# SJTU-IPADS/wukong

Hardware: AMD Instinct MI355X
Metric: queries/sec, LUBM-2560 Q1-Q7 mix (OSDI16 plans) (higher is better)
Workload: dtype u32

## Files before the change

wukong_amd/csrc/gpu_engine.hip:

```cpp
#include "wk_store.h"
#include "../../include/wukong_abi.h"

#include <hip/hip_runtime.h>

#include <vector>
#include <algorithm>
#include <cstring>
#include <cstdio>
#include <cstdlib>
#include <chrono>
#include <type_traits>

static double now_us() {
    return std::chrono::duration<double, std::micro>(
               std::chrono::steady_clock::now().time_since_epoch()).count();
}
static int wk_verbose_lvl() {
    static int v = -1;
    if (v < 0) { const char *e = getenv("WK_VERBOSE"); v = e ? atoi(e) : 0; }
    return v;
}

using namespace wk;

// ... 138 lines not shown
    int nvars = 0;
    int step = 0;
    struct fconj { std::vector<wk_fnode_t> prog; int after; };
    std::vector<wk_fnode_t> filt;
    std::vector<fconj> conj;

    struct wk_graph {
        hipGraphExec_t exec = nullptr;
        std::vector<int32_t> v2c;
        int ncols = 0, cur = 0, nvars = 0;
        int64_t bound = 0;
        bool light = false;
        const sid_t *view = nullptr;
        bool fin = false;
        fin_sig_t fin_sig;
    };
    std::vector<wk_graph> graphs;
    int capturing = 0;
    std::vector<uint8_t> capture_hint;
    int capture_empty_after = -1;

    bool timing = false;
    std::vector<timed_launch> pending;
    double cat_usec[CAT_COUNT] = {0};
    double cat_bytes[CAT_COUNT] = {0};
    int64_t cat_n[CAT_COUNT] = {0};

    int var2col(ssid_t v) const { return v < 0 ? v2c[-(v + 1)] : -1; }
    int var_stat(ssid_t v) const { return v >= 0 ? 2 : (var2col(v) >= 0 ? 1 : 0); }
};

static const int BLOCK = 256;
static_assert(BLOCK == SCAN_T, "kernels declare __launch_bounds__(SCAN_T)");
static inline const sid_t *cur_table(wk_engine *e);
static int grid_for(int64_t work) {
    int64_t g = (work + BLOCK - 1) / BLOCK;
    return (int)(g < 1 ? 1 : (g > 2048 ? 2048 : g));
}
static inline const sid_t *cur_table(wk_engine *e) {
    return e->tbl_view ? e->tbl_view : (const sid_t *)e->tbl[e->cur].p;
}
static int32_t materialize_view(wk_engine *e) {
    if (!e->tbl_view) return WK_OK;
    size_t bytes = (size_t)std::max<int64_t>(e->nrows, 0) *
                   std::max(e->ncols, 1) * 4;
    if (bytes &&
        hipMemcpyAsync(e->tbl[e->cur].p, e->tbl_view, bytes,
                       hipMemcpyDeviceToDevice, e->stream) != hipSuccess)
        return WK_ERR_HIP;
    e->tbl_view = nullptr;
    return WK_OK;
}
static inline void fin_invalidate(wk_engine *e) {
    e->fin_count = -1;
    e->fin_table = false;
}
static int fin_grid(int64_t cap_rows) {
    int64_t g = (cap_rows + BLOCK - 1) / BLOCK;
    return (int)(g < 1 ? 1 : (g > FIN_MAXB ? FIN_MAXB : g));
}
static int scan_grid(int64_t bound) {
    int64_t g = (bound + SCAN_T) / SCAN_T + 1;
    return (int)(g < 1 ? 1 : (g > 2048 ? 2048 : g));
}

static hipEvent_t ev_get() { hipEvent_t e; (void)hipEventCreate(&e); return e; }

static bool wk_fn_dispatch() {
    const char *v = getenv("WK_FN_DISPATCH");
    return !(v && !atoi(v));
}

static bool wk_row_chain() {
    const char *v = getenv("WK_ROW_CHAIN");
    return !(v && v[0] == '0');
}
static bool wk_chain() {
    const char *v = getenv("WK_CHAIN");
    return !(v && !atoi(v));
}
static bool chain_narrow(int out_cols) {
    const char *v = getenv("WK_CHAIN_WIDTH");
    return out_cols <= ROW_NARROW && !(v && atoi(v) == ROW_MAX);
}
static bool wk_filter_batch() {
    const char *v = getenv("WK_FILTER_BATCH");
    return !(v && !atoi(v));
}
static bool wk_wave_scan() {
    const char *v = getenv("WK_SCAN");
    return !(v && !atoi(v));
}

static bool wk_filter_pushdown() {
    const char *v = getenv("WK_FILTER_PUSHDOWN");
    return !(v && !atoi(v));
}

static bool wk_spin_sync() {
    static int v = -1;
    if (v < 0) { const char *e = getenv("WK_SPIN_SYNC"); v = e ? atoi(e) : 0; }
    return v;
}
static hipError_t stream_sync(hipStream_t s) {
    if (!wk_spin_sync()) return hipStreamSynchronize(s);
    hipError_t rc;
    while ((rc = hipStreamQuery(s)) == hipErrorNotReady) {}
    return rc;
}

#define TIME_BEGIN(eng)                                                     \
    hipEvent_t t_s_ = nullptr, t_e_ = nullptr;                              \
    if ((eng)->timing && !(eng)->capturing) {                               \
        t_s_ = ev_get(); t_e_ = ev_get();                                   \
        (void)hipEventRecord(t_s_, (eng)->stream); }

#define TIME_END(eng, category)                                             \
    if ((eng)->timing && !(eng)->capturing) {                               \
        (void)hipEventRecord(t_e_, (eng)->stream);                          \
        (eng)->pending.push_back({t_s_, t_e_, (category)}); }

static const char *CAT_NAMES[CAT_COUNT] = {"probe", "scan", "expand", "filter",
                                           "copy", "split", "other"};

static void resolve_timing(wk_engine *e) {
    for (auto &t : e->pending) {
        float ms = 0;
        (void)hipEventElapsedTime(&ms, t.start, t.stop);
        if (wk_verbose_lvl() >= 3)
            fprintf(stderr, "[launch] %s %.0fus\n", CAT_NAMES[t.cat], ms * 1e3);
        e->cat_usec[t.cat] += ms * 1000.0;
        e->cat_n[t.cat]++;
        (void)hipEventDestroy(t.start);
        (void)hipEventDestroy(t.stop);
    }
    e->pending.clear();
}

static int64_t min_cap_rows() {
    const char *v = getenv("WK_MIN_CAP");
    return v ? atoll(v) : (1 << 20);
}

static int32_t grow_caps(wk_engine *e, int64_t rows, int cols) {
    rows = std::max<int64_t>(rows, min_cap_rows());
    cols = std::max(cols, std::max(e->cap_cols, 1));
    if (rows <= e->cap_rows && cols <= e->cap_cols) return WK_OK;
    if (e->capturing) return WK_ERR_STATE;
    rows = std::max(rows, e->cap_rows);
    HIP_CHECK(stream_sync(e->stream));
    fin_invalidate(e);
    size_t keep = (size_t)std::max<int64_t>(e->nrows, 0) * std::max(e->ncols, 0) * 4;
    keep = std::min(keep, e->tbl[e->cur].cap);
    void *saved = nullptr;
    if (keep) {
        if (hipMalloc(&saved, keep) != hipSuccess) return WK_ERR_HIP;
        HIP_CHECK(hipMemcpy(saved, e->tbl[e->cur].p, keep, hipMemcpyDeviceToDevice));
    }
    if (e->tbl[0].ensure((size_t)rows * cols * 4)) return WK_ERR_HIP;
    if (e->tbl[1].ensure((size_t)rows * cols * 4)) return WK_ERR_HIP;
    if (saved) {
        HIP_CHECK(hipMemcpy(e->tbl[e->cur].p, saved, keep, hipMemcpyDeviceToDevice));
        (void)hipFree(saved);
    }
    if (e->cnt.ensure((size_t)(rows + 1) * 4)) return WK_ERR_HIP;
    if (e->pmask.ensure((size_t)(rows + 1) * 4)) return WK_ERR_HIP;
// ... 519 lines not shown
    if (e->h_pin[S_ERR]) {
        e->h_pin[7] = 0;
        return WK_ERR_CAP;
    }
    return WK_OK;
}

static int32_t sync_state_grow(wk_engine *e) {
    int32_t rc = sync_state(e);
    if (rc != WK_ERR_CAP) return rc;
    int64_t need = (int64_t)e->h_pin[S_REQ];
    e->nrows = 0;
    int32_t rc2 = grow_caps(e, need + need / 4, e->cap_cols);
    if (rc2) return rc2;
    e->zero_pending = true;
    return WK_ERR_CAP;
}

template <class F>
static void with_ncols(int ncols, F &&f) {
    switch (ncols) {
    case 1: f(std::integral_constant<int, 1>{}); break;
    case 2: f(std::integral_constant<int, 2>{}); break;
    case 3: f(std::integral_constant<int, 3>{}); break;
    case 4: f(std::integral_constant<int, 4>{}); break;
    case 5: f(std::integral_constant<int, 5>{}); break;
    case 6: f(std::integral_constant<int, 6>{}); break;
    case 7: f(std::integral_constant<int, 7>{}); break;
    default: f(std::integral_constant<int, 8>{}); break;
    }
}


static bool hint_nodrop(const wk_engine *e, int step) {
    return e->capturing && step < (int)e->capture_hint.size() &&
           e->capture_hint[step];
}

static sid_t typeof_lookahead(const wk_engine *e, ssid_t o) {
    if (e->step + 1 >= (int)e->pats.size()) return 0;
    const wk_pattern_t &nx = e->pats[e->step + 1];
    if (nx.subject == o && nx.predicate == (ssid_t)TYPE_ID &&
        nx.direction == DIR_OUT && nx.object > 0)
        return (sid_t)nx.object;
    return 0;
}

static const uint64_t *type_bitmap(const wk_engine *e, sid_t type_id) {
    return (e->gs && (size_t)type_id < e->gs->d_tbm.size())
               ? e->gs->d_tbm[type_id]
               : nullptr;
}

static const fnpage_t *fn_map(const wk_engine *e, ssid_t p, int dir,
                              const sid_t **vals) {
    const size_t w = (size_t)p * 2 + dir;
    if (!e->gs || w >= e->gs->d_fn_pages.size() || !e->gs->d_fn_pages[w])
        return nullptr;
    *vals = e->gs->d_fn_vals[w];
    return e->gs->d_fn_pages[w];
}

struct chain_plan {
    chain_t C{};
    int npat = 0;
    int nfilter = 0;
    int out_cols = 0;
    int nnew = 0;
    ssid_t new_vars[CHAIN_MAX];
    bool lone_typeof(int col) const {
        return npat == 1 && C.op[0].kind == CH_TYPE && C.op[0].a == col;
    }
};

static bool chain_enabled(const wk_engine *e) {
    return e->whole_plan && !e->hinting && !e->opt_mode &&
           e->remote_step_idx < 0 && e->gs && wk_fn_dispatch() && wk_chain();
}

static void collect_chain(const wk_engine *e, int from,
                          std::vector<int32_t> v2c, int ncols,
                          chain_plan &cp) {
    const wk_store *st = e->st;
    cp.C.fn_base = st->fn_base;
    cp.C.fn_n = st->fn_n;
    cp.C.t_base = st->type_base;
    cp.C.t_n = st->type_n;
    int end = (int)e->pats.size();
    if (e->capturing && e->capture_empty_after >= 0)
        end = std::min(end, e->capture_empty_after + 1);
    auto col_of = [&](ssid_t v) {
        const int i = -(v + 1);
        return (v < 0 && i < (int)v2c.size()) ? v2c[i] : -1;
    };
    for (int i = from; i < end && cp.npat < CHAIN_MAX; i++) {
        const wk_pattern_t &pt = e->pats[i];
        const ssid_t p = pt.predicate;
        const int dir = pt.direction;
        const int a = col_of(pt.subject);
        if (a < 0 || p < 1) break;
        if ((sid_t)p == TYPE_ID && dir == DIR_IN) break;
        chain_op op{nullptr, nullptr, 0, a, 0, 0};
        const sid_t *vals = nullptr;
        if (pt.object >= 0) {
            if ((sid_t)p == TYPE_ID && dir == DIR_OUT) {
                const uint64_t *tbm = type_bitmap(e, (sid_t)pt.object);
                if (!tbm) break;
                op.kind = CH_TYPE;
                op.data = tbm;
            } else {
                if (fn_map(e, p, dir, &vals) || st->nsrv != 1 ||
                    !fn_map(e, p, dir ^ 1, &vals))
                    break;
                op.kind = CH_EQ;
                op.cval = st->fn_get((size_t)p * 2 + (dir ^ 1),
                                     (sid_t)pt.object);
            }
            cp.nfilter++;
        } else if (col_of(pt.object) >= 0) {
            op.kind = CH_FN_EQ;
            op.b = col_of(pt.object);
            op.pg = fn_map(e, p, dir, &vals);
            if (!op.pg && st->nsrv == 1) {
                op.pg = fn_map(e, p, dir ^ 1, &vals);
                std::swap(op.a, op.b);
            }
            if (!op.pg) break;
            op.data = vals;
            cp.nfilter++;
        } else {
            const int oi = -(pt.object + 1);
            if (oi >= (int)v2c.size() || ncols + 1 > e->cap_cols ||
                ncols + 1 > ROW_MAX)
                break;
            op.pg = fn_map(e, p, dir, &vals);
            if (!op.pg) break;
            op.kind = CH_FN_APPEND;
            op.data = vals;
            v2c[oi] = ncols++;
            cp.new_vars[cp.nnew++] = pt.object;
        }
        cp.C.op[cp.npat++] = op;
    }
    cp.C.nops = cp.npat;
    cp.out_cols = ncols;
}

static void bind_chain_vars(wk_engine *e, const chain_plan &cp, int first_col) {
    for (int j = 0; j < cp.nnew; j++)
        e->v2c[-(cp.new_vars[j] + 1)] = first_col + j;
}

static void finish_step_in_place(wk_engine *e, ssid_t new_var, int out_cols,
                                 int64_t bound, int consumed) {
    if (new_var < 0) e->v2c[-(new_var + 1)] = e->ncols;
    fin_invalidate(e);
    e->ncols = out_cols;
    e->bound = bound;
    e->step += consumed;
}
static void finish_step(wk_engine *e, ssid_t new_var, int out_cols,
                        int64_t bound, int consumed) {
    finish_step_in_place(e, new_var, out_cols, bound, consumed);
    e->cur ^= 1;
    e->tbl_view = nullptr;
}

static void launch_commit(wk_engine *e) {
    hipLaunchKernelGGL(k_commit, dim3(1), dim3(1), 0, e->stream, e->d_state,
                       (uint64_t)e->cap_rows);
}

static fparams fparams_list(const wk_engine *e, const sid_t *edges,
                            const sid_t *cur_tbl, int col, int dir,
                            uint64_t off, uint64_t sz) {
    return fparams{e->d_verts, edges, 0, 1, cur_tbl, e->ncols, col, 0u,
                   dir, PK_NORMAL, PM_LIST, 0, 0u, off, sz, e->d_type_of,
                   0, 0, 0, nullptr, nullptr, nullptr, 0, 0, 0};
}
static void launch_filter_tpr(wk_engine *e, const fparams &P, int verify_only,
                              sid_t *out_tbl) {
    hipLaunchKernelGGL(k_filter_tpr, dim3(grid_for(e->bound)), dim3(BLOCK), 0,
                       e->stream, P, verify_only, (int)wk_filter_batch(),
                       e->d_state, e->d_stats, out_tbl);
}

static void launch_scan_mid(wk_engine *e, int G) {
    hipLaunchKernelGGL(wk_wave_scan() ? k_scan_mid : k_scan_mid_ladder,
                       dim3(1), dim3(SCAN_T), 0, e->stream,
                       (uint64_t *)e->bsums.p, G, (uint64_t)e->cap_rows,
                       e->d_state);
}
template <class Gather>
static void launch_gather_scan(wk_engine *e, int G, bool timed,
                               Gather &&gather) {
    auto front = [&] {
        gather();
        hipLaunchKernelGGL(wk_wave_scan() ? k_scan_local : k_scan_local_ladder,
                           dim3(G), dim3(SCAN_T), 0, e->stream,
                           (const uint32_t *)e->cnt.p, e->d_state,
                           (uint64_t *)e->prefix.p, (uint64_t *)e->bsums.p);
    };
    if (!timed) {
        front();
        launch_scan_mid(e, G);
        return;
    }
    {
        TIME_BEGIN(e);
        front();
        TIME_END(e, CAT_PROBE);
    }
    {
        TIME_BEGIN(e);
        launch_scan_mid(e, G);
        TIME_END(e, CAT_SCAN);
    }
}

struct expand_verify {
    const uint64_t *tbm = nullptr;
    const uint16_t *type_of = nullptr;
    uint64_t base = 0, n = 0;
    sid_t cval = 0;
    int on = 0;
};

template <int NC>
// ... 376 lines not shown
    finish_step(e, c.o, e->ncols + 1, e->bound, fuse ? 2 : 1);
    return WK_OK;
}

static int32_t step_k2u_tf(wk_engine *e, const step_ctx &c,
                           const fnpage_t *c_pg, const uint64_t *tf_tbm) {
    const wk_store *st = e->st;
    const int G = scan_grid(e->bound);
    launch_gather_scan(e, G,  true, [&] {
        hipLaunchKernelGGL(k_csr_gather_tf, dim3(grid_for(e->bound)),
                           dim3(BLOCK), 0, e->stream, c.cur_tbl, e->ncols,
                           c.col, c_pg,
                           e->gs->d_csr_entries[(size_t)c.p * 2 + c.dir],
                           st->fn_base, st->fn_n, e->d_edges, tf_tbm,
                           st->type_base, st->type_n, e->d_state, e->d_stats,
                           (uint64_t *)e->eoff.p, (uint32_t *)e->cnt.p);
    });
    {
        TIME_BEGIN(e);
        launch_expand_tf(e, c.cur_tbl, c.out_tbl, G, tf_tbm);
        TIME_END(e, CAT_EXPAND);
    }
    finish_step(e, c.o, e->ncols + 1, e->cap_rows, 2);
    return WK_OK;
}

static int32_t step_k2u_classic(wk_engine *e, const step_ctx &c,
                                const fnpage_t *c_pg) {
    const wk_store *st = e->st;
    const int G = scan_grid(e->bound);
    if (c_pg) {
        launch_gather_scan(e, G,  true, [&] {
            hipLaunchKernelGGL(k_csr_gather, dim3(grid_for(e->bound)),
                               dim3(BLOCK), 0, e->stream, c.cur_tbl, e->ncols,
                               c.col, c_pg,
                               e->gs->d_csr_entries[(size_t)c.p * 2 + c.dir],
                               st->fn_base, st->fn_n, e->d_state, e->d_stats,
                               (uint64_t *)e->eoff.p, (uint32_t *)e->cnt.p);
        });
    } else {
        {
            TIME_BEGIN(e);
            hipLaunchKernelGGL(k_probe_scan, dim3(G), dim3(SCAN_T), 0,
                               e->stream, e->d_verts, c.cur_tbl, e->ncols,
                               c.col, (uint32_t)c.p, c.dir, c.key_mode,
                               c.seg->bucket_start, c.seg->num_buckets,
                               e->d_state, e->d_stats, (uint64_t *)e->eoff.p,
                               (uint32_t *)e->cnt.p, (uint64_t *)e->prefix.p,
                               (uint64_t *)e->bsums.p);
            TIME_END(e, CAT_PROBE);
        }
        {
            TIME_BEGIN(e);
            launch_scan_mid(e, G);
            TIME_END(e, CAT_SCAN);
        }
    }
    expand_verify vf;
    if (hint_nodrop(e, e->step + 1) && st->nsrv == 1)
        vf.cval = typeof_lookahead(e, c.o);
    if (vf.cval) {
        vf.base = st->type_base;
        vf.n = st->type_n;
        vf.tbm = type_bitmap(e, vf.cval);
        vf.type_of = e->d_type_of;
        if (vf.tbm || vf.type_of) vf.on = 1;
    }
    {
        TIME_BEGIN(e);
        launch_expand(e, c.cur_tbl, c.out_tbl, G, vf);
        TIME_END(e, CAT_EXPAND);
    }
    finish_step(e, c.o, e->ncols + 1, e->cap_rows, vf.on ? 2 : 1);
    return WK_OK;
}

template <int NC, int W>
static void launch_k2u_chain(wk_engine *e, const step_ctx &c,
                             const fnpage_t *c_pg, const chain_plan &cp,
                             int G) {
    const wk_store *st = e->st;
    launch_gather_scan(e, G,  true, [&] {
        hipLaunchKernelGGL(
            (k_csr_gather_chain<NC, W>), dim3(grid_for(e->bound)),
            dim3(BLOCK), 0, e->stream, c.cur_tbl, c.col, c_pg,
            e->gs->d_csr_entries[(size_t)c.p * 2 + c.dir], st->fn_base,
            st->fn_n, e->d_edges, cp.C, e->d_state, e->d_stats,
            (uint64_t *)e->eoff.p, (uint32_t *)e->cnt.p,
            (uint32_t *)e->pmask.p);
    });
    TIME_BEGIN(e);
    hipLaunchKernelGGL(
        (k_expand_chain<NC, W>), dim3(grid_for(e->bound)), dim3(BLOCK), 0,
        e->stream, c.cur_tbl, e->d_edges, (uint64_t *)e->eoff.p,
        (uint32_t *)e->cnt.p, (uint32_t *)e->pmask.p,
        (uint64_t *)e->prefix.p,
        (uint64_t *)e->bsums.p, G, cp.C, cp.out_cols, e->d_state,
        (uint64_t)e->cap_rows, e->d_stats, (uint32_t *)e->ovf.p,
        c.out_tbl);
    hipLaunchKernelGGL(
        k_expand_chain_big<NC>, dim3(512), dim3(BLOCK), 0, e->stream,
        c.cur_tbl, e->d_edges, (uint64_t *)e->eoff.p,
        (uint64_t *)e->prefix.p, (uint64_t *)e->bsums.p, G, cp.C,
        cp.out_cols, e->d_state, (uint64_t)e->cap_rows,
        (uint32_t *)e->ovf.p, c.out_tbl);
    TIME_END(e, CAT_EXPAND);
}
static int32_t step_k2u_chain(wk_engine *e, const step_ctx &c,
                              const fnpage_t *c_pg, const chain_plan &cp) {
    const int G = scan_grid(e->bound);
    const int nc_in = e->ncols;
    if (nc_in + 1 > ROW_MAX) return WK_ERR_STATE;
    const bool narrow = chain_narrow(cp.out_cols);
    with_ncols(nc_in, [&](auto nc) {
        constexpr int NC = decltype(nc)::value;
        if constexpr (NC < ROW_NARROW) {
            if (narrow) {
                launch_k2u_chain<NC, ROW_NARROW>(e, c, c_pg, cp, G);
                return;
            }
        }
        if constexpr (NC < ROW_MAX)
            launch_k2u_chain<NC, ROW_MAX>(e, c, c_pg, cp, G);
    });
    bind_chain_vars(e, cp, nc_in + 1);
    finish_step(e, c.o, cp.out_cols, e->cap_rows, 1 + cp.npat);
    return WK_OK;
}

template <int NC, int W>
static void launch_row_chain(wk_engine *e, const step_ctx &c,
                             const chain_plan &cp) {
    hipLaunchKernelGGL((k_row_chain<NC, W>), dim3(grid_for(e->bound)),
                       dim3(BLOCK), 0, e->stream, c.cur_tbl, cp.C,
                       cp.out_cols, e->d_state, (uint64_t)e->cap_rows,
                       e->d_stats, c.out_tbl);
}
static int32_t step_row_chain(wk_engine *e, const step_ctx &c,
                              const chain_plan &cp) {
    const int nc_in = e->ncols;
    const bool narrow = chain_narrow(cp.out_cols);
    TIME_BEGIN(e);
    with_ncols(nc_in, [&](auto nc) {
        constexpr int NC = decltype(nc)::value;
        if constexpr (NC <= ROW_NARROW) {
            if (narrow) {
                launch_row_chain<NC, ROW_NARROW>(e, c, cp);
                return;
            }
        }
        launch_row_chain<NC, ROW_MAX>(e, c, cp);
    });
    TIME_END(e, CAT_FILTER);
    launch_commit(e);
    bind_chain_vars(e, cp, nc_in);
    finish_step(e, 0, cp.out_cols, e->bound, cp.npat);
    return WK_OK;
}

static int32_t step_k2u(wk_engine *e, const step_ctx &c) {
    const wk_store *st = e->st;
    if (e->ncols + 1 > e->cap_cols) return WK_ERR_STATE;
    const size_t w_seg = (size_t)c.p * 2 + c.dir;
    const bool side = c.key_mode == PK_NORMAL && e->gs && wk_fn_dispatch();
    if (side && !e->gs->d_fn_pages.empty() && e->gs->d_fn_pages[w_seg])
        return step_k2u_fn(e, c, e->gs->d_fn_pages[w_seg],
                           e->gs->d_fn_vals[w_seg]);
    const fnpage_t *c_pg = (side && !e->gs->d_csr_pages.empty())
                               ? e->gs->d_csr_pages[w_seg]
                               : nullptr;
    const bool tf_deg_ok =
        w_seg < st->seg_keys.size() && st->seg_keys[w_seg] &&
        st->seg_edges[w_seg] / st->seg_keys[w_seg] <= 32;
    if (c_pg && tf_deg_ok && st->nsrv == 1 && chain_enabled(e)) {
        chain_plan cp;
        std::vector<int32_t> v2c = e->v2c;
        v2c[-(c.o + 1)] = e->ncols;
        collect_chain(e, e->step + 1, v2c, e->ncols + 1, cp);
        if (cp.nfilter && !cp.lone_typeof(e->ncols))
            return step_k2u_chain(e, c, c_pg, cp);
    }
    if (c_pg && tf_deg_ok && st->nsrv == 1 && !e->hinting &&
        !hint_nodrop(e, e->step + 1)) {
        const sid_t t = typeof_lookahead(e, c.o);
        const uint64_t *tf_tbm = t ? type_bitmap(e, t) : nullptr;
        if (tf_tbm) return step_k2u_tf(e, c, c_pg, tf_tbm);
    }
    return step_k2u_classic(e, c, c_pg);
}

static int32_t exec_pattern(wk_engine *e) {
    if (!e || e->step >= (int)e->pats.size()) return WK_ERR_STATE;
    const wk_store *st = e->st;
    const wk_pattern_t pat = e->pats[e->step];
    const bool index_start =
        (e->step == 0 && pat.subject >= 0 && is_tpid(pat.subject));
    const bool start =
        e->step != e->remote_step_idx && !e->opt_mode && pat.predicate >= 0 &&
        (index_start || (pat.subject >= 0 && pat.object < 0 &&
                         e->var2col(pat.object) < 0));
    if (!start) flush_begin(e);
    if (e->step == e->remote_step_idx) return exec_pattern_remote(e);
    if (e->opt_mode && e->tbl_view) {
        int32_t rcm = materialize_view(e);
        if (rcm) return rcm;
    }
    step_ctx c{pat.subject, pat.predicate, pat.object, pat.direction,
               cur_table(e), (sid_t *)e->tbl[e->cur ^ 1].p};
    if (e->opt_mode) return step_optional(e, c);
    if (c.p < 0) return step_versatile(e, c);

    if (start) return step_start(e, c, index_start);
    if (c.s >= 0) return step_const_to_known(e, c);

    c.col = e->var2col(c.s);
    if (c.col < 0) return WK_ERR_PLAN;
// ... 1193 lines not shown
```

wukong_amd/csrc/wk_kernels_common.h:

```cpp
#pragma once


enum { PK_NORMAL = 0, PK_INDEX = 1 };
enum { PM_SIZE = 0,
       PM_CONST = 1,
       PM_COL = 2,
       PM_LIST = 3,
       PM_EQ = 4 };

enum { S_NROWS = 0, S_TOTAL = 1, S_ERR = 2, S_REQ = 3, S_OVF = 4,
       S_DONE = 5, S_INROWS = 6, S_WORDS = 7 };
enum { CAT_PROBE = 0, CAT_SCAN, CAT_EXPAND, CAT_FILTER, CAT_COPY, CAT_SPLIT,
       CAT_OTHER, CAT_COUNT };

constexpr int SCAN_T = 256;

__device__ __forceinline__ void count_bytes(uint64_t *stats, int cat,
                                            uint64_t bytes) {
    if (blockIdx.x == 0 && threadIdx.x == 0 && stats)
        atomicAdd((unsigned long long *)&stats[cat], (unsigned long long)bytes);
}

__device__ __forceinline__ bool bsearch_u32(const sid_t *a, uint64_t n, sid_t x) {
    uint64_t lo = 0, hi = n;
    while (lo < hi) {
        uint64_t mid = (lo + hi) >> 1;
        sid_t v = a[mid];
        if (v < x) lo = mid + 1;
        else if (v > x) hi = mid;
        else return true;
    }
    return false;
}

__device__ __forceinline__ bool tbm_has(const uint64_t *__restrict__ tbm,
                                        uint64_t base, uint64_t n, sid_t v) {
    const uint64_t ix = (uint64_t)v - base;
    return ix < n && ((tbm[ix >> 6] >> (ix & 63)) & 1);
}

__device__ __forceinline__ uint64_t csr_entry(const fnpage_t *__restrict__ pg,
                                              const uint64_t *__restrict__ entries,
                                              uint64_t base, uint64_t n,
                                              sid_t v) {
    const uint32_t rk = rank_lookup(pg, base, n, v);
    return rk == RANK_MISS ? 0 : entries[rk];
}

__device__ __forceinline__ bool typeof_nodrop_ok(
    const uint64_t *__restrict__ tbm, const uint16_t *__restrict__ type_of,
    uint64_t base, uint64_t n, sid_t cval, sid_t v) {
    if (tbm) return tbm_has(tbm, base, n, v);
    const uint64_t tix = (uint64_t)v - base;
    const uint16_t t = (tix < n) ? type_of[tix] : 0;
    return t != 0xFFFF && (sid_t)t == cval;
}

enum { CH_FN_APPEND = 0,
       CH_TYPE = 1,
       CH_FN_EQ = 2,
       CH_EQ = 3 };
constexpr int CHAIN_MAX = 8;
constexpr int ROW_MAX = 8;
constexpr int ROW_NARROW = 4;
constexpr int CHAIN_EK = 4;
constexpr int CHAIN_RPT = 2;

struct chain_op {
    const fnpage_t *pg;
    const void *data;
    int32_t kind, a, b;
    sid_t cval;
};
struct chain_t {
    chain_op op[CHAIN_MAX];
    uint64_t fn_base, fn_n, t_base, t_n;
    int32_t nops;
};

__device__ __forceinline__ sid_t row_get(const sid_t (&row)[ROW_MAX], int c) {
    sid_t v = row[0];
#pragma unroll
    for (int i = 1; i < ROW_MAX; i++) v = (c == i) ? row[i] : v;
    return v;
}
template <int W>
__device__ __forceinline__ void row_set(sid_t (&row)[W], int c, sid_t v) {
#pragma unroll
    for (int i = 0; i < W; i++) row[i] = (c == i) ? v : row[i];
}

template <int NC>
__device__ __forceinline__ bool chain_eval(const chain_t &C,
                                           sid_t (&row)[ROW_MAX]) {
    int nc = NC;
#pragma unroll
    for (int i = 0; i < CHAIN_MAX; i++) {
        if (i >= C.nops) break;
        const chain_op &o = C.op[i];
        const sid_t v = row_get(row, o.a);
        if (o.kind == CH_TYPE) {
            if (!tbm_has((const uint64_t *)o.data, C.t_base, C.t_n, v))
                return false;
        } else if (o.kind == CH_EQ) {
            if (v != o.cval) return false;
        } else {
            const sid_t tv = fn_lookup(o.pg, (const sid_t *)o.data, C.fn_base,
                                       C.fn_n, v);
            if (!tv) return false;
            if (o.kind == CH_FN_EQ) {
                if (tv != row_get(row, o.b)) return false;
            } else {
                row_set(row, nc++, tv);
            }
        }
    }
    return true;
}

template <int W>
__device__ __forceinline__ sid_t row_pick(const sid_t (&row)[W], int c) {
    sid_t v = 0;
#pragma unroll
    for (int i = 0; i < W; i++) v |= row[i] & (0u - (sid_t)(c == i));
    return v;
}

template <int NC, int K, bool APPEND_ONLY = false, int W = ROW_MAX>
__device__ __forceinline__ uint32_t chain_eval_batch(
    const chain_t &C, sid_t (&rows)[K][W], uint32_t active) {
    static_assert(K >= 1 && K <= 32, "keep mask is 32 bits");
    static_assert(NC <= W && W <= ROW_MAX, "the input columns must fit");
    uint32_t keep = active;
    int nc = NC;
#pragma unroll 1
    for (int i = 0; i < C.nops; i++) {
        const chain_op &o = C.op[i];
        if (o.kind == CH_TYPE) {
            if (APPEND_ONLY) continue;
            const uint64_t *tbm = (const uint64_t *)o.data;
            if (!tbm || !C.t_n) { keep = 0; continue; }
            uint64_t ix[K], w[K];
#pragma unroll
            for (int j = 0; j < K; j++) {
                const uint64_t x = (uint64_t)row_pick(rows[j], o.a) - C.t_base;
                const bool ok = ((keep >> j) & 1) && x < C.t_n;
                keep = ok ? keep : keep & ~(1u << j);
                ix[j] = ok ? x : 0;
            }
#pragma unroll
            for (int j = 0; j < K; j++) w[j] = tbm[ix[j] >> 6];
#pragma unroll
            for (int j = 0; j < K; j++)
                keep = ((w[j] >> (ix[j] & 63)) & 1) ? keep : keep & ~(1u << j);
        } else if (o.kind == CH_EQ) {
            if (APPEND_ONLY) continue;
#pragma unroll
            for (int j = 0; j < K; j++)
                keep = (row_pick(rows[j], o.a) == o.cval) ? keep
                                                          : keep & ~(1u << j);
        } else {
            if (APPEND_ONLY && o.kind != CH_FN_APPEND) continue;
            const sid_t *vals = (const sid_t *)o.data;
            if (!o.pg || !vals || !C.fn_n) {
                keep = 0;
                if (o.kind == CH_FN_APPEND) nc++;
                continue;
            }
            uint64_t ix[K], bits[K];
            uint32_t rk[K];
            sid_t tv[K];
#pragma unroll
            for (int j = 0; j < K; j++) {
                const uint64_t x = (uint64_t)row_pick(rows[j], o.a) - C.fn_base;
                const bool ok = ((keep >> j) & 1) && x < C.fn_n;
                keep = ok ? keep : keep & ~(1u << j);
                ix[j] = ok ? x : 0;
            }
#pragma unroll
            for (int j = 0; j < K; j++) {
                const uint4 q =
                    *reinterpret_cast<const uint4 *>(&o.pg[ix[j] >> 6]);
                bits[j] = (uint64_t)q.x | ((uint64_t)q.y << 32);
                rk[j] = q.z;
            }
#pragma unroll
            for (int j = 0; j < K; j++) {
                const uint64_t bit = 1ull << (ix[j] & 63);
                const bool hit = ((keep >> j) & 1) && (bits[j] & bit);
                keep = hit ? keep : keep & ~(1u << j);
                rk[j] = hit ? rk[j] + (uint32_t)__popcll(bits[j] & (bit - 1))
                            : 0u;
            }
#pragma unroll
            for (int j = 0; j < K; j++) tv[j] = vals[rk[j]];
            if (o.kind == CH_FN_EQ) {
#pragma unroll
                for (int j = 0; j < K; j++)
                    keep = (tv[j] && tv[j] == row_pick(rows[j], o.b))
                               ? keep
                               : keep & ~(1u << j);
            } else {
#pragma unroll
                for (int j = 0; j < K; j++) {
                    keep = tv[j] ? keep : keep & ~(1u << j);
                    row_set(rows[j], nc, tv[j]);
                }
                nc++;
            }
        }
    }
    return keep;
}

__device__ __forceinline__ void probe_one(const vertex_t *__restrict__ verts,
                                          uint64_t bucket_start,
                                          uint64_t num_buckets, uint64_t key,
                                          uint64_t &eoff, uint64_t &esz) {
    uint64_t bucket = bucket_start + hash_u64(key) % num_buckets;
    while (true) {
        const vertex_t *b = &verts[bucket * ASSOC];
        uint64_t k0 = b[0].key, k1 = b[1].key, k2 = b[2].key, k3 = b[3].key;
        uint64_t k4 = b[4].key, k5 = b[5].key, k6 = b[6].key, k7 = b[7].key;
        int hit = -1;
        if (k0 == key) hit = 0;
        else if (k1 == key) hit = 1;
        else if (k2 == key) hit = 2;
        else if (k3 == key) hit = 3;
        else if (k4 == key) hit = 4;
        else if (k5 == key) hit = 5;
        else if (k6 == key) hit = 6;
        if (hit >= 0) {
            uint64_t pp = b[hit].ptr;
            eoff = ptr_off(pp);
            esz = ptr_size(pp);
            return;
        }
        if (k7 == KEY_EMPTY) { eoff = 0; esz = 0; return; }
        bucket = key_vid(k7);
    }
}

__device__ __forceinline__ void probe_chain(const vertex_t *__restrict__ verts,
                                            uint64_t bucket, uint64_t key,
                                            uint64_t &eoff, uint64_t &esz) {
    while (true) {
        const vertex_t *b = &verts[bucket * ASSOC];
        int hit = -1;
#pragma unroll
        for (int i = 0; i < ASSOC - 1; i++)
            if (b[i].key == key && hit < 0) hit = i;
        if (hit >= 0) {
            eoff = ptr_off(b[hit].ptr);
            esz = ptr_size(b[hit].ptr);
            return;
        }
        if (b[ASSOC - 1].key == KEY_EMPTY) { eoff = 0; esz = 0; return; }
        bucket = key_vid(b[ASSOC - 1].key);
    }
}
```

wukong_amd/csrc/wk_kernels_expand.h:

```cpp
#pragma once

__global__ void k_probe_scan(const vertex_t *__restrict__ verts,
                             const sid_t *__restrict__ tbl, int ncols,
                             int col, uint32_t pid, int dir, int key_mode,
                             uint64_t bucket_start, uint64_t num_buckets,
                             uint64_t *__restrict__ d_state,
                             uint64_t *__restrict__ d_stats,
                             uint64_t *__restrict__ d_eoff,
                             uint32_t *__restrict__ d_cnt,
                             uint64_t *__restrict__ d_pre,
                             uint64_t *__restrict__ bsums)
{
    const int64_t nrows = (int64_t)d_state[S_NROWS];
    count_bytes(d_stats, CAT_PROBE, (uint64_t)nrows * (4 + 128 + 8 + 12));
    const int64_t chunk = (nrows + gridDim.x - 1) / gridDim.x;
    const int64_t start = (int64_t)blockIdx.x * chunk;
    const int64_t end = min(start + chunk, nrows);
    __shared__ uint64_t sh[SCAN_T];
    uint64_t carry = 0;

    auto key_of = [&](int64_t r) {
        sid_t v = tbl[r * ncols + col];
        return (key_mode == PK_NORMAL) ? key_pack(v, pid, (uint64_t)dir)
                                       : key_pack(0, v, (uint64_t)dir);
// ... 357 lines not shown
                act |= on ? 1u << j : 0u;
#pragma unroll
                for (int c = 0; c < W; c++) cand[j][c] = 0;
#pragma unroll
                for (int c = 0; c < NC; c++) cand[j][c] = in[c];
                cand[j][NC] = edges[off + p];
            }
            if (oc > NC + 1)
                act = chain_eval_batch<NC + 1, EK, true>(C, cand, act);
#pragma unroll
            for (int j = 0; j < EK; j++) {
                if (((act >> j) & 1) && basep + w < cap) {
#pragma unroll
                    for (int c = 0; c < W; c++)
                        if (c < oc) dst[c] = cand[j][c];
                    dst += oc;
                    w++;
                }
            }
        }
    }
    if (blockIdx.x == 0 && threadIdx.x == 0)
        atomicAdd((unsigned long long *)&d_stats[CAT_EXPAND],
                  (unsigned long long)(d_state[S_NROWS] * (4 * oc) +
                                       (uint64_t)nrows * 24));
}

template <int NC>
__global__ void k_expand_chain_big(const sid_t *__restrict__ tbl,
                                   const sid_t *__restrict__ edges,
                                   const uint64_t *__restrict__ d_eoff,
                                   const uint64_t *__restrict__ d_pre,
                                   const uint64_t *__restrict__ bsums, int G,
                                   chain_t C, int oc,
                                   const uint64_t *__restrict__ d_state,
                                   uint64_t cap,
                                   const uint32_t *__restrict__ ovf,
                                   sid_t *__restrict__ out)
{
    static_assert(NC < ROW_MAX, "the edge value needs a column");
    const int64_t nq = (int64_t)d_state[S_OVF];
    const int64_t nrows = (int64_t)d_state[S_INROWS];
    const int64_t chunk = (nrows + G - 1) / G;
    const int lane = threadIdx.x & 63;
    const int64_t w0 = ((int64_t)blockIdx.x * blockDim.x + threadIdx.x) >> 6;
    const int64_t nw = ((int64_t)gridDim.x * blockDim.x) >> 6;
    for (int64_t q = w0; q < nq; q += nw) {
        const int64_t r = ovf[q];
        const uint64_t e = d_eoff[r];
        const uint64_t off = csr_off(e);
        const uint32_t len = csr_len(e);
        uint64_t basep = d_pre[r] + bsums[r / chunk];
        if (basep >= cap) continue;
        sid_t row[ROW_MAX];
#pragma unroll
        for (int c = 0; c < ROW_MAX; c++) row[c] = 0;
#pragma unroll
        for (int c = 0; c < NC; c++) row[c] = tbl[r * NC + c];
        uint64_t wbase = 0;
        for (uint32_t k0 = 0; k0 < len; k0 += 64) {
            const uint32_t k = k0 + lane;
            bool pass = false;
            if (k < len) {
                row[NC] = edges[off + k];
                pass = chain_eval<NC + 1>(C, row);
            }
            uint64_t mask = __ballot(pass);
            if (pass) {
                uint64_t pos = basep + wbase +
                               (uint64_t)__popcll(mask & ((1ull << lane) - 1));
                if (pos < cap) {
                    sid_t *dst = out + (int64_t)pos * oc;
#pragma unroll
                    for (int c = 0; c < ROW_MAX; c++)
                        if (c < oc) dst[c] = row[c];
                }
            }
            wbase += (uint64_t)__popcll(mask);
        }
    }
}

template <int NC, int W>
__global__ void __launch_bounds__(SCAN_T)
k_row_chain(const sid_t *__restrict__ tbl, chain_t C, int oc,
            uint64_t *__restrict__ d_state, uint64_t cap,
            uint64_t *__restrict__ d_stats, sid_t *__restrict__ out)
{
    static_assert(NC <= W && W <= ROW_MAX, "the input columns must fit");
    constexpr int K = 4;
    const int64_t nrows = (int64_t)d_state[S_NROWS];
    count_bytes(d_stats, CAT_FILTER, (uint64_t)nrows * (4 * NC + 4 * oc));
    __shared__ unsigned long long s_base;
    __shared__ unsigned int s_cnt;
    __shared__ unsigned int s_wbase[SCAN_T / 64];
    const int lane = threadIdx.x & 63;
    const int wid = threadIdx.x >> 6;
    const int64_t tile = (int64_t)SCAN_T * K;
    const int64_t stride = (int64_t)gridDim.x * tile;
    for (int64_t base = (int64_t)blockIdx.x * tile; base < nrows;
         base += stride) {
        sid_t rows[K][W];
        uint32_t active = 0;
#pragma unroll
        for (int k = 0; k < K; k++) {
            const int64_t r = base + k * SCAN_T + threadIdx.x;
            const bool in = r < nrows;
            const int64_t rr = in ? r : base;
            active |= in ? 1u << k : 0u;
#pragma unroll
            for (int c = 0; c < W; c++) rows[k][c] = 0;
#pragma unroll
            for (int c = 0; c < NC; c++) rows[k][c] = tbl[rr * NC + c];
        }
        const uint32_t keep = chain_eval_batch<NC, K>(C, rows, active);
        if (threadIdx.x == 0) s_cnt = 0;
        __syncthreads();
        uint64_t mask[K];
        uint32_t wtot = 0;
#pragma unroll
        for (int k = 0; k < K; k++) {
            mask[k] = __ballot((keep >> k) & 1);
            wtot += (uint32_t)__popcll(mask[k]);
        }
        if (lane == 0) s_wbase[wid] = atomicAdd(&s_cnt, wtot);
        __syncthreads();
        if (threadIdx.x == 0)
            s_base = s_cnt ? atomicAdd((unsigned long long *)&d_state[S_TOTAL],
                                       (unsigned long long)s_cnt)
                           : 0;
        __syncthreads();
        uint64_t wpos = s_base + s_wbase[wid];
#pragma unroll
        for (int k = 0; k < K; k++) {
            const uint64_t pos =
                wpos + (uint32_t)__popcll(mask[k] & ((1ull << lane) - 1));
            if (((keep >> k) & 1) && pos < cap) {
                sid_t *dst = out + (int64_t)pos * oc;
#pragma unroll
                for (int c = 0; c < W; c++)
                    if (c < oc) dst[c] = rows[k][c];
            }
            wpos += (uint32_t)__popcll(mask[k]);
        }
    }
}

__device__ __forceinline__ uint64_t wave_incl_scan(uint64_t v, int lane) {
#pragma unroll
    for (int ofs = 1; ofs < 64; ofs <<= 1) {
        const uint64_t t = __shfl_up((unsigned long long)v, ofs);
        if (lane >= ofs) v += t;
    }
    return v;
}

__device__ __forceinline__ uint64_t block_excl_scan(uint64_t tsum,
                                                    uint64_t (*s_wtot)[SCAN_T / 64],
                                                    int par, uint64_t *total) {
    static_assert(SCAN_T == 256, "four wave totals");
    const int lane = threadIdx.x & 63, wid = threadIdx.x >> 6;
    const uint64_t incl = wave_incl_scan(tsum, lane);
    if (lane == 63) s_wtot[par][wid] = incl;
    __syncthreads();
    const uint64_t w0 = s_wtot[par][0], w1 = s_wtot[par][1],
                   w2 = s_wtot[par][2], w3 = s_wtot[par][3];
    const uint64_t wbase = (wid > 0 ? w0 : 0) + (wid > 1 ? w1 : 0) +
// ... 444 lines not shown
```

Baseline: 19320.

## Schedule chain ops into two-slot rounds with paired loads and early exit

Adds a host-side scheduler that packs independent chain filter/append ops into rounds of two slots, so the gather loads of two independent ops are issued together and their memory latency overlaps. Ops that do not depend on each other share a round. It also adds a wave-wide early exit when no row survives. Chain kernel grids are capped at the resident occupancy computed via the occupancy API, and launch bounds are raised for narrow row-chain variants. This increases the number of template instantiations and register pressure, and the per-round switch adds branching.

```diff
diff --git a/wukong_amd/csrc/gpu_engine.hip b/wukong_amd/csrc/gpu_engine.hip
--- a/wukong_amd/csrc/gpu_engine.hip
+++ b/wukong_amd/csrc/gpu_engine.hip
@@ -244,6 +244,28 @@
 static bool chain_narrow(int out_cols) {
     const char *v = getenv("WK_CHAIN_WIDTH");
     return out_cols <= ROW_NARROW && !(v && atoi(v) == ROW_MAX);
+}
+static bool wk_chain_sched() {
+    const char *v = getenv("WK_CHAIN_SCHED");
+    return !(v && !atoi(v));
+}
+template <auto Kern>
+static int chain_grid(int64_t work) {
+    static const int resident = [] {
+        int nb = 0, dev = 0, cus = 0;
+        if (hipGetDevice(&dev) != hipSuccess ||
+            hipDeviceGetAttribute(&cus, hipDeviceAttributeMultiprocessorCount,
+                                  dev) != hipSuccess ||
+            hipOccupancyMaxActiveBlocksPerMultiprocessor(&nb, Kern, BLOCK,
+                                                         0) != hipSuccess ||
+            nb < 1 || cus < 1)
+            return 2048;
+        return std::min(2048, nb * cus);
+    }();
+    int g = std::min(grid_for(work), resident);
+    const char *v = getenv("WK_CHAIN_GRID");
+    const int cap = v ? atoi(v) : 0;
+    return cap > 0 && cap < g ? cap : g;
 }
 static bool wk_filter_batch() {
     const char *v = getenv("WK_FILTER_BATCH");
@@ -929,6 +951,7 @@
                           std::vector<int32_t> v2c, int ncols,
                           chain_plan &cp) {
     const wk_store *st = e->st;
+    const int nc_in = ncols;
     cp.C.fn_base = st->fn_base;
     cp.C.fn_n = st->fn_n;
     cp.C.t_base = st->type_base;
@@ -947,7 +970,7 @@
         const int a = col_of(pt.subject);
         if (a < 0 || p < 1) break;
         if ((sid_t)p == TYPE_ID && dir == DIR_IN) break;
-        chain_op op{nullptr, nullptr, 0, a, 0, 0};
+        chain_op op{nullptr, nullptr, 0, a, 0, 0, -1};
         const sid_t *vals = nullptr;
         if (pt.object >= 0) {
             if ((sid_t)p == TYPE_ID && dir == DIR_OUT) {
@@ -991,6 +1014,18 @@
     }
     cp.C.nops = cp.npat;
     cp.out_cols = ncols;
+    chain_sched_op sop[CHAIN_MAX];
+    for (int i = 0; i < cp.npat; i++)
+        sop[i] = {cp.C.op[i].kind, cp.C.op[i].a, cp.C.op[i].b};
+    chain_sched S;
+    chain_schedule(sop, cp.npat, nc_in, wk_chain_sched(), S);
+    cp.C.nrounds = S.nrounds;
+    cp.C.early_out = S.early_out;
+    for (int i = 0; i < CHAIN_MAX; i++) {
+        cp.C.op[i].dst = S.dst[i];
+        for (int s2 = 0; s2 < CHAIN_SLOTS; s2++)
+            cp.C.slot[i][s2] = S.slot[i][s2];
+    }
 }
 
 static void bind_chain_vars(wk_engine *e, const chain_plan &cp, int first_col) {
@@ -1533,7 +1568,8 @@
     const wk_store *st = e->st;
     launch_gather_scan(e, G,  true, [&] {
         hipLaunchKernelGGL(
-            (k_csr_gather_chain<NC, W>), dim3(grid_for(e->bound)),
+            (k_csr_gather_chain<NC, W>),
+            dim3(chain_grid<k_csr_gather_chain<NC, W>>(e->bound)),
             dim3(BLOCK), 0, e->stream, c.cur_tbl, c.col, c_pg,
             e->gs->d_csr_entries[(size_t)c.p * 2 + c.dir], st->fn_base,
             st->fn_n, e->d_edges, cp.C, e->d_state, e->d_stats,
@@ -1542,7 +1578,8 @@
     });
     TIME_BEGIN(e);
     hipLaunchKernelGGL(
-        (k_expand_chain<NC, W>), dim3(grid_for(e->bound)), dim3(BLOCK), 0,
+        (k_expand_chain<NC, W>),
+        dim3(chain_grid<k_expand_chain<NC, W>>(e->bound)), dim3(BLOCK), 0,
         e->stream, c.cur_tbl, e->d_edges, (uint64_t *)e->eoff.p,
         (uint32_t *)e->cnt.p, (uint32_t *)e->pmask.p,
         (uint64_t *)e->prefix.p,
@@ -1582,7 +1619,8 @@
 template <int NC, int W>
 static void launch_row_chain(wk_engine *e, const step_ctx &c,
                              const chain_plan &cp) {
-    hipLaunchKernelGGL((k_row_chain<NC, W>), dim3(grid_for(e->bound)),
+    hipLaunchKernelGGL((k_row_chain<NC, W>),
+                       dim3(chain_grid<k_row_chain<NC, W>>(e->bound)),
                        dim3(BLOCK), 0, e->stream, c.cur_tbl, cp.C,
                        cp.out_cols, e->d_state, (uint64_t)e->cap_rows,
                        e->d_stats, c.out_tbl);
diff --git a/wukong_amd/csrc/wk_chain_sched.h b/wukong_amd/csrc/wk_chain_sched.h
--- /dev/null
+++ b/wukong_amd/csrc/wk_chain_sched.h
@@ -0,0 +1,52 @@
+#pragma once
+#include <cstdint>
+
+enum { CH_FN_APPEND = 0,
+       CH_TYPE = 1,
+       CH_FN_EQ = 2,
+       CH_EQ = 3 };
+constexpr int CHAIN_MAX = 8;
+constexpr int CHAIN_SLOTS = 2;
+
+struct chain_sched_op {
+    int32_t kind, a, b;
+};
+struct chain_sched {
+    int32_t nrounds;
+    int32_t slot[CHAIN_MAX][CHAIN_SLOTS];
+    int32_t dst[CHAIN_MAX];
+    int32_t round_of[CHAIN_MAX];
+    int32_t early_out;
+};
+
+inline void chain_schedule(const chain_sched_op *ops, int nops, int nc_in,
+                           bool packed, chain_sched &S) {
+    S.nrounds = 0;
+    S.early_out = packed ? 1 : 0;
+    int fill[CHAIN_MAX];
+    for (int r = 0; r < CHAIN_MAX; r++) {
+        fill[r] = 0;
+        S.dst[r] = S.round_of[r] = -1;
+        for (int s = 0; s < CHAIN_SLOTS; s++) S.slot[r][s] = -1;
+    }
+    int nc = nc_in;
+    for (int i = 0; i < nops && i < CHAIN_MAX; i++) {
+        int r = 0;
+        if (!packed) {
+            r = i;
+        } else {
+            for (int j = 0; j < i; j++) {
+                if (ops[j].kind != CH_FN_APPEND) continue;
+                const bool reads =
+                    ops[i].a == S.dst[j] ||
+                    (ops[i].kind == CH_FN_EQ && ops[i].b == S.dst[j]);
+                if (reads && S.round_of[j] + 1 > r) r = S.round_of[j] + 1;
+            }
+            while (fill[r] == CHAIN_SLOTS) r++;
+        }
+        S.slot[r][fill[r]++] = i;
+        S.round_of[i] = r;
+        if (ops[i].kind == CH_FN_APPEND) S.dst[i] = nc++;
+        if (r + 1 > S.nrounds) S.nrounds = r + 1;
+    }
+}
diff --git a/wukong_amd/csrc/wk_kernels_common.h b/wukong_amd/csrc/wk_kernels_common.h
--- a/wukong_amd/csrc/wk_kernels_common.h
+++ b/wukong_amd/csrc/wk_kernels_common.h
@@ -1,4 +1,5 @@
 #pragma once
+#include "wk_chain_sched.h"
 
 
 enum { PK_NORMAL = 0, PK_INDEX = 1 };
@@ -56,11 +57,6 @@
     return t != 0xFFFF && (sid_t)t == cval;
 }
 
-enum { CH_FN_APPEND = 0,
-       CH_TYPE = 1,
-       CH_FN_EQ = 2,
-       CH_EQ = 3 };
-constexpr int CHAIN_MAX = 8;
 constexpr int ROW_MAX = 8;
 constexpr int ROW_NARROW = 4;
 constexpr int CHAIN_EK = 4;
@@ -71,11 +67,14 @@
     const void *data;
     int32_t kind, a, b;
     sid_t cval;
+    int32_t dst;
 };
 struct chain_t {
     chain_op op[CHAIN_MAX];
     uint64_t fn_base, fn_n, t_base, t_n;
-    int32_t nops;
+    int32_t nops, nrounds;
+    int32_t early_out;
+    int32_t slot[CHAIN_MAX][CHAIN_SLOTS];
 };
 
 __device__ __forceinline__ sid_t row_get(const sid_t (&row)[ROW_MAX], int c) {
@@ -126,57 +125,28 @@
     return v;
 }
 
-template <int NC, int K, bool APPEND_ONLY = false, int W = ROW_MAX>
-__device__ __forceinline__ uint32_t chain_eval_batch(
-    const chain_t &C, sid_t (&rows)[K][W], uint32_t active) {
-    static_assert(K >= 1 && K <= 32, "keep mask is 32 bits");
-    static_assert(NC <= W && W <= ROW_MAX, "the input columns must fit");
-    uint32_t keep = active;
-    int nc = NC;
-#pragma unroll 1
-    for (int i = 0; i < C.nops; i++) {
-        const chain_op &o = C.op[i];
-        if (o.kind == CH_TYPE) {
-            if (APPEND_ONLY) continue;
+enum { SL_NONE = 0, SL_BITS = 1, SL_MAP = 2 };
+
+template <int M, int K, int W>
+__device__ __forceinline__ void chain_slot_load(
+    const chain_t &C, const chain_op &o, const sid_t (&rows)[K][W],
+    uint32_t &keep, uint32_t (&ix)[K], uint64_t (&bits)[K],
+    uint32_t (&rk)[K]) {
+    if constexpr (M != SL_NONE) {
+        const uint64_t base = M == SL_BITS ? C.t_base : C.fn_base;
+        const uint64_t n = M == SL_BITS ? C.t_n : C.fn_n;
+#pragma unroll
+        for (int j = 0; j < K; j++) {
+            const uint64_t x = (uint64_t)row_pick(rows[j], o.a) - base;
+            const bool ok = ((keep >> j) & 1) && x < n;
+            keep = ok ? keep : keep & ~(1u << j);
+            ix[j] = ok ? (uint32_t)x : 0u;
+        }
+        if constexpr (M == SL_BITS) {
             const uint64_t *tbm = (const uint64_t *)o.data;
-            if (!tbm || !C.t_n) { keep = 0; continue; }
-            uint64_t ix[K], w[K];
-#pragma unroll
-            for (int j = 0; j < K; j++) {
-                const uint64_t x = (uint64_t)row_pick(rows[j], o.a) - C.t_base;
-                const bool ok = ((keep >> j) & 1) && x < C.t_n;
-                keep = ok ? keep : keep & ~(1u << j);
-                ix[j] = ok ? x : 0;
-            }
-#pragma unroll
-            for (int j = 0; j < K; j++) w[j] = tbm[ix[j] >> 6];
-#pragma unroll
-            for (int j = 0; j < K; j++)
-                keep = ((w[j] >> (ix[j] & 63)) & 1) ? keep : keep & ~(1u << j);
-        } else if (o.kind == CH_EQ) {
-            if (APPEND_ONLY) continue;
-#pragma unroll
-            for (int j = 0; j < K; j++)
-                keep = (row_pick(rows[j], o.a) == o.cval) ? keep
-                                                          : keep & ~(1u << j);
+#pragma unroll
+            for (int j = 0; j < K; j++) bits[j] = tbm[ix[j] >> 6];
         } else {
-            if (APPEND_ONLY && o.kind != CH_FN_APPEND) continue;
-            const sid_t *vals = (const sid_t *)o.data;
-            if (!o.pg || !vals || !C.fn_n) {
-                keep = 0;
-                if (o.kind == CH_FN_APPEND) nc++;
-                continue;
-            }
-            uint64_t ix[K], bits[K];
-            uint32_t rk[K];
-            sid_t tv[K];
-#pragma unroll
-            for (int j = 0; j < K; j++) {
-                const uint64_t x = (uint64_t)row_pick(rows[j], o.a) - C.fn_base;
-                const bool ok = ((keep >> j) & 1) && x < C.fn_n;
-                keep = ok ? keep : keep & ~(1u << j);
-                ix[j] = ok ? x : 0;
-            }
 #pragma unroll
             for (int j = 0; j < K; j++) {
                 const uint4 q =
@@ -184,31 +154,117 @@
                 bits[j] = (uint64_t)q.x | ((uint64_t)q.y << 32);
                 rk[j] = q.z;
             }
-#pragma unroll
-            for (int j = 0; j < K; j++) {
-                const uint64_t bit = 1ull << (ix[j] & 63);
-                const bool hit = ((keep >> j) & 1) && (bits[j] & bit);
-                keep = hit ? keep : keep & ~(1u << j);
-                rk[j] = hit ? rk[j] + (uint32_t)__popcll(bits[j] & (bit - 1))
-                            : 0u;
-            }
-#pragma unroll
-            for (int j = 0; j < K; j++) tv[j] = vals[rk[j]];
-            if (o.kind == CH_FN_EQ) {
+        }
+    }
+}
+template <int M, int K>
+__device__ __forceinline__ void chain_slot_mid(
+    const chain_op &o, uint32_t &keep, const uint32_t (&ix)[K],
+    const uint64_t (&bits)[K], uint32_t (&rk)[K]) {
+    if constexpr (M == SL_BITS) {
+#pragma unroll
+        for (int j = 0; j < K; j++)
+            keep = ((bits[j] >> (ix[j] & 63)) & 1) ? keep : keep & ~(1u << j);
+    } else if constexpr (M == SL_MAP) {
+        const sid_t *vals = (const sid_t *)o.data;
+#pragma unroll
+        for (int j = 0; j < K; j++) {
+            const uint64_t bit = 1ull << (ix[j] & 63);
+            const bool hit = ((keep >> j) & 1) && (bits[j] & bit);
+            keep = hit ? keep : keep & ~(1u << j);
+            rk[j] = hit ? rk[j] + (uint32_t)__popcll(bits[j] & (bit - 1)) : 0u;
+        }
+#pragma unroll
+        for (int j = 0; j < K; j++) rk[j] = vals[rk[j]];
+    }
+}
+template <int M, int K, int W>
+__device__ __forceinline__ void chain_slot_end(const chain_op &o,
+                                               sid_t (&rows)[K][W],
+                                               uint32_t &keep,
+                                               const uint32_t (&tv)[K]) {
+    if constexpr (M == SL_MAP) {
+        const bool eq = o.kind == CH_FN_EQ;
+        const int dst = eq ? -1 : o.dst;
+#pragma unroll
+        for (int j = 0; j < K; j++) {
+            const bool ok = tv[j] && (!eq || tv[j] == row_pick(rows[j], o.b));
+            keep = ok ? keep : keep & ~(1u << j);
+            row_set(rows[j], dst, tv[j]);
+        }
+    }
+}
+template <int M0, int M1, int K, int W>
+__device__ __forceinline__ uint32_t chain_round(const chain_t &C,
+                                                const chain_op &o0,
+                                                const chain_op &o1,
+                                                sid_t (&rows)[K][W],
+                                                uint32_t keep) {
+    uint32_t ix0[K], ix1[K], rk0[K], rk1[K];
+    uint64_t b0[K], b1[K];
+    chain_slot_load<M0>(C, o0, rows, keep, ix0, b0, rk0);
+    chain_slot_load<M1>(C, o1, rows, keep, ix1, b1, rk1);
+    chain_slot_mid<M0>(o0, keep, ix0, b0, rk0);
+    chain_slot_mid<M1>(o1, keep, ix1, b1, rk1);
+    chain_slot_end<M0>(o0, rows, keep, rk0);
+    chain_slot_end<M1>(o1, rows, keep, rk1);
+    return keep;
+}
+
+template <int NC, int K, bool APPEND_ONLY = false, int W = ROW_MAX>
+__device__ __forceinline__ uint32_t chain_eval_batch(
+    const chain_t &C, sid_t (&rows)[K][W], uint32_t active) {
+    static_assert(K >= 1 && K <= 32, "keep mask is 32 bits");
+    static_assert(NC <= W && W <= ROW_MAX, "the input columns must fit");
+    static_assert(CHAIN_SLOTS == 2, "chain_round takes two slots");
+    uint32_t keep = active;
+#pragma unroll 1
+    for (int r = 0; r < C.nrounds; r++) {
+        int idx[2], cls[2];
+#pragma unroll
+        for (int s = 0; s < 2; s++) {
+            const int i = C.slot[r][s];
+            idx[s] = i < 0 ? 0 : i;
+            const chain_op &o = C.op[idx[s]];
+            cls[s] = SL_NONE;
+            if (i < 0 || (APPEND_ONLY && o.kind != CH_FN_APPEND)) continue;
+            if (o.kind == CH_EQ) {
 #pragma unroll
                 for (int j = 0; j < K; j++)
-                    keep = (tv[j] && tv[j] == row_pick(rows[j], o.b))
+                    keep = (row_pick(rows[j], o.a) == o.cval)
                                ? keep
                                : keep & ~(1u << j);
+            } else if (o.kind == CH_TYPE) {
+                if (o.data && C.t_n) cls[s] = SL_BITS;
+                else keep = 0;
             } else {
-#pragma unroll
-                for (int j = 0; j < K; j++) {
-                    keep = tv[j] ? keep : keep & ~(1u << j);
-                    row_set(rows[j], nc, tv[j]);
-                }
-                nc++;
+                if (o.pg && o.data && C.fn_n) cls[s] = SL_MAP;
+                else keep = 0;
             }
         }
+        const bool sw = cls[0] < cls[1];
+        const chain_op &o0 = C.op[sw ? idx[1] : idx[0]];
+        const chain_op &o1 = C.op[sw ? idx[0] : idx[1]];
+        switch ((sw ? cls[1] : cls[0]) * 3 + (sw ? cls[0] : cls[1])) {
+        case SL_MAP * 3 + SL_MAP:
+            keep = chain_round<SL_MAP, SL_MAP>(C, o0, o1, rows, keep);
+            break;
+        case SL_MAP * 3 + SL_BITS:
+            keep = chain_round<SL_MAP, SL_BITS>(C, o0, o1, rows, keep);
+            break;
+        case SL_MAP * 3 + SL_NONE:
+            keep = chain_round<SL_MAP, SL_NONE>(C, o0, o1, rows, keep);
+            break;
+        case SL_BITS * 3 + SL_BITS:
+            keep = chain_round<SL_BITS, SL_BITS>(C, o0, o1, rows, keep);
+            break;
+        case SL_BITS * 3 + SL_NONE:
+            keep = chain_round<SL_BITS, SL_NONE>(C, o0, o1, rows, keep);
+            break;
+        default:
+            break;
+        }
+        if (!APPEND_ONLY && C.early_out && __ballot(keep != 0) == 0) break;
     }
     return keep;
 }
diff --git a/wukong_amd/csrc/wk_kernels_expand.h b/wukong_amd/csrc/wk_kernels_expand.h
--- a/wukong_amd/csrc/wk_kernels_expand.h
+++ b/wukong_amd/csrc/wk_kernels_expand.h
@@ -463,7 +463,8 @@
 }
 
 template <int NC, int W>
-__global__ void __launch_bounds__(SCAN_T)
+__global__ void
+__launch_bounds__(SCAN_T, W == ROW_NARROW && NC <= 2 ? 8 : 1)
 k_row_chain(const sid_t *__restrict__ tbl, chain_t C, int oc,
             uint64_t *__restrict__ d_state, uint64_t cap,
             uint64_t *__restrict__ d_stats, sid_t *__restrict__ out)
```

Result: faster. 20040 (median of 6 runs) (+3.7%).
